# yangcaoai/CoDA_NeurIPS2023

Measured on NVIDIA H100. Metric: training scenes/sec (20k-pt SUN-RGBD synth, 256 queries), higher is better.
Workload: dtype fp32

## Files before the change

### coda_neurips2023_b200/csrc/gemm_tn32_sm90.cu

```cuda
#include "../../include/coda_gemm.h"
#include "a32_prologue.cuh"
#include "sm90_primitives.cuh"

using namespace coda;

namespace {

constexpr int BM = 128;
constexpr int BKR = 32;
constexpr int NS = 2;
constexpr int RAW_STAGES = 2, PL_STAGES = 3;
constexpr int TW = 8;
constexpr int TN32_THREADS = 288;

struct TN32Maps {
  CUtensorMap a, a2, b;
};

struct TN32Params {
  long long rows;
  int m, n;
  int a_mode, b_mode;
  const float *a_scale, *a_shift, *a_alpha, *a_beta;
  const float *dpooled;
  const unsigned char *argmax;
  int group;
  const float *b_scale, *b_shift;
  float *a_colsum;
  float *partial;
  float *c;
  long long ldc;
  int ksplit;
};

template <int BN>
__global__ void __launch_bounds__(TN32_THREADS, 1)
gemm_tn32_kernel(const __grid_constant__ TN32Maps maps, const TN32Params P) {
  constexpr int RAW_A = BKR * BM * 4;
  constexpr int RAW_B = BKR * BN * 4;
  constexpr int RAW_X = 1024;
  constexpr int RAW_STAGE = 2 * RAW_A + RAW_B + RAW_X;
  constexpr int PL_A = BKR * BM * 2;
  constexpr int PL_B = BKR * BN * 2;
  constexpr int PL_STAGE = NS * (PL_A + PL_B);
  extern __shared__ __align__(1024) unsigned char smem_raw[];
  unsigned char *smem = smem_align1024(smem_raw);
  unsigned char *raw_ring = smem;
  unsigned char *pl_ring = smem + (size_t)RAW_STAGES * RAW_STAGE;
  __shared__ __align__(8) uint64_t raw_full[RAW_STAGES], raw_empty[RAW_STAGES];
  __shared__ __align__(16) float s_colsum[TW][BM];

  const int warp = threadIdx.x >> 5, lane = threadIdx.x & 31;
  const int tiles_n = (P.n + BN - 1) / BN;
  const int tile = blockIdx.x / P.ksplit, ks = blockIdx.x % P.ksplit;
  const int m0 = (tile / tiles_n) * BM, n0 = (tile % tiles_n) * BN;
  const long long nkb_total = (P.rows + BKR - 1) / BKR;
  const long long per = (nkb_total + P.ksplit - 1) / P.ksplit;
  const long long kb0 = (long long)ks * per;
  const long long nkb = max(0ll, min(per, nkb_total - kb0));
  const bool two_in = P.a_mode == CODA_A32_BN_BWD;

  if (threadIdx.x == 0) {
    for (int s = 0; s < RAW_STAGES; ++s) { mbar_init(&raw_full[s], 1); mbar_init(&raw_empty[s], TW); }
    mbar_fence_init_cluster();
  }
  __syncthreads();

  if (warp == 8) {
    if (lane == 0) {
      prefetch_tmap(&maps.a);
      prefetch_tmap(&maps.b);
      if (two_in) prefetch_tmap(&maps.a2);
    }
    const bool pooled = P.a_mode == CODA_A32_BN_BWD_POOLED || P.a_mode == CODA_A32_BN_BWD_POOLED_PRE;
    const uint32_t bytes = (uint32_t)(RAW_A * (two_in ? 2 : 1) + RAW_B + (pooled ? 640 : 0));
    const long long ngroups = pooled ? P.rows / P.group : 0;
    for (long long i = 0; i < nkb; ++i) {
      const int rs = (int)(i % RAW_STAGES);
      mbar_wait(&raw_empty[rs], (uint32_t)((i / RAW_STAGES) & 1) ^ 1u);
      if (elect_one_sync()) {
        unsigned char *st = raw_ring + (size_t)rs * RAW_STAGE;
        const int r0 = (int)((kb0 + i) * BKR);
        mbar_arrive_expect_tx(&raw_full[rs], bytes);
        if (pooled) {
          long long g = (long long)r0 / P.group;
          if (g >= ngroups) g = ngroups - 1;
          bulk_load_1d(st + 2 * RAW_A + RAW_B, P.dpooled + g * P.m + m0, 512, &raw_full[rs]);
          bulk_load_1d(st + 2 * RAW_A + RAW_B + 512, P.argmax + g * P.m + m0, 128, &raw_full[rs]);
        }
#pragma unroll
        for (int g = 0; g < BM / 32; ++g) tma_load_3d(st + g * 4096, &maps.a, &raw_full[rs], m0 + g * 32, r0, 0);
        if (two_in) {
#pragma unroll
          for (int g = 0; g < BM / 32; ++g) tma_load_3d(st + RAW_A + g * 4096, &maps.a2, &raw_full[rs], m0 + g * 32, r0, 0);
        }
#pragma unroll
        for (int g = 0; g < BN / 32; ++g) tma_load_3d(st + 2 * RAW_A + g * 4096, &maps.b, &raw_full[rs], n0 + g * 32, r0, 0);
      }
      __syncwarp();
    }
    return;
  }

  const int tw = warp;
  const int wg = warp >> 2;
  const bool want_colsum = P.a_colsum != nullptr && n0 == 0;
  float4 csum = make_float4(0.f, 0.f, 0.f, 0.f);
  const int ca = m0 + lane * 4;
  float4 sa = make_float4(0.f, 0.f, 0.f, 0.f), ta = sa, al = sa, be = sa;
  if (P.a_mode != CODA_A32_PLAIN && ca < P.m) {
    sa = __ldg(reinterpret_cast<const float4 *>(P.a_scale + ca));
    ta = __ldg(reinterpret_cast<const float4 *>(P.a_shift + ca));
    al = __ldg(reinterpret_cast<const float4 *>(P.a_alpha + ca));
    be = __ldg(reinterpret_cast<const float4 *>(P.a_beta + ca));
  }
  constexpr int B_CHUNKS = BN / 4, B_RPP = 32 / B_CHUNKS;
  const int bch = lane % B_CHUNKS, brow_off = lane / B_CHUNKS;
  const int cb = n0 + bch * 4;
  float4 sb = make_float4(0.f, 0.f, 0.f, 0.f), tb = sb;
  if (P.b_mode == CODA_A32_AFFINE_RELU && cb < P.n) {
    sb = __ldg(reinterpret_cast<const float4 *>(P.b_scale + cb));
    tb = __ldg(reinterpret_cast<const float4 *>(P.b_shift + cb));
  }
  const bool a_col_ok = ca < P.m;
  const bool pooled_mode = P.a_mode == CODA_A32_BN_BWD_POOLED || P.a_mode == CODA_A32_BN_BWD_POOLED_PRE;
  int rem0 = pooled_mode ? (int)((kb0 * BKR) % P.group) : 0;
  int rs = 0, ps = 0;
  uint32_t raw_par = 0;
  float acc[BN / 2];
  for (long long i = 0; i < nkb; ++i) {
    mbar_wait_relaxed(&raw_full[rs], raw_par);
    const unsigned char *raw = raw_ring + (size_t)rs * RAW_STAGE;
    unsigned char *pl = pl_ring + (size_t)ps * PL_STAGE;
    const long long r0 = (kb0 + i) * BKR;
    const bool tail = r0 + BKR > P.rows;
#pragma unroll
      for (int j = 0; j < BKR / TW; ++j) {
        const int r = tw + j * TW;
        const long long grow = r0 + r;
        const uint32_t roff = (uint32_t)(lane >> 3) * 4096u + (uint32_t)r * 128u + (uint32_t)(((lane & 7) ^ (r & 7)) << 4);
        float4 y = *reinterpret_cast<const float4 *>(raw + roff);
        float4 o = y;
        if (P.a_mode == CODA_A32_BN_BWD) {
          const float4 d = *reinterpret_cast<const float4 *>(raw + RAW_A + roff);
          o.x = a32::bn_bwd(y.x, d.x, sa.x, ta.x, al.x, be.x);
          o.y = a32::bn_bwd(y.y, d.y, sa.y, ta.y, al.y, be.y);
          o.z = a32::bn_bwd(y.z, d.z, sa.z, ta.z, al.z, be.z);
          o.w = a32::bn_bwd(y.w, d.w, sa.w, ta.w, al.w, be.w);
        } else if (P.a_mode == CODA_A32_BN_BWD_POOLED_PRE) {
          const int gi = rem0 + r;
          const float4 d = *reinterpret_cast<const float4 *>(raw + 2 * RAW_A + RAW_B + lane * 16);
          const uchar4 id = *reinterpret_cast<const uchar4 *>(raw + 2 * RAW_A + RAW_B + 512 + lane * 4);
          o.x = a32::bn_bwd_pooled_pre(y.x, d.x, id.x == gi, al.x, be.x);
          o.y = a32::bn_bwd_pooled_pre(y.y, d.y, id.y == gi, al.y, be.y);
          o.z = a32::bn_bwd_pooled_pre(y.z, d.z, id.z == gi, al.z, be.z);
          o.w = a32::bn_bwd_pooled_pre(y.w, d.w, id.w == gi, al.w, be.w);
        } else if (P.a_mode == CODA_A32_BN_BWD_POOLED) {
          const int gi = rem0 + r;
          const float4 d = *reinterpret_cast<const float4 *>(raw + 2 * RAW_A + RAW_B + lane * 16);
          const uchar4 id = *reinterpret_cast<const uchar4 *>(raw + 2 * RAW_A + RAW_B + 512 + lane * 4);
          o.x = a32::bn_bwd_pooled(y.x, d.x, id.x == gi, sa.x, ta.x, al.x, be.x);
          o.y = a32::bn_bwd_pooled(y.y, d.y, id.y == gi, sa.y, ta.y, al.y, be.y);
          o.z = a32::bn_bwd_pooled(y.z, d.z, id.z == gi, sa.z, ta.z, al.z, be.z);
          o.w = a32::bn_bwd_pooled(y.w, d.w, id.w == gi, sa.w, ta.w, al.w, be.w);
        }
        if (tail && grow >= P.rows) o = make_float4(0.f, 0.f, 0.f, 0.f);
        if (want_colsum) { csum.x += o.x; csum.y += o.y; csum.z += o.z; csum.w += o.w; }
        const int col = lane * 4;
        split_store4<NS>(o, reinterpret_cast<__nv_bfloat16 *>(pl + (col >> 6) * (BKR * 128) + r * 128 +
                                                              ((((col & 63) >> 3) ^ (r & 7)) << 4) + ((col & 7) >> 2) * 8),
                         PL_A / 2);
      }
#pragma unroll
      for (int j = 0; j < BKR / (TW * B_RPP); ++j) {
        const int r = (tw + j * TW) * B_RPP + brow_off;
        const long long grow = r0 + r;
        const uint32_t roff = (uint32_t)(bch >> 3) * 4096u + (uint32_t)r * 128u + (uint32_t)(((bch & 7) ^ (r & 7)) << 4);
        float4 v = *reinterpret_cast<const float4 *>(raw + 2 * RAW_A + roff);
        if (P.b_mode == CODA_A32_AFFINE_RELU) {
          v.x = a32::affine_relu(v.x, sb.x, tb.x); v.y = a32::affine_relu(v.y, sb.y, tb.y);
          v.z = a32::affine_relu(v.z, sb.z, tb.z); v.w = a32::affine_relu(v.w, sb.w, tb.w);
        }
        if (tail && grow >= P.rows) v = make_float4(0.f, 0.f, 0.f, 0.f);
        const int col = bch * 4;
        split_store4<NS>(v, reinterpret_cast<__nv_bfloat16 *>(pl + NS * PL_A + (col >> 6) * (BKR * 128) + r * 128 +
                                                              ((((col & 63) >> 3) ^ (r & 7)) << 4) + ((col & 7) >> 2) * 8),
                         PL_B / 2);
      }
      fence_proxy_async_smem();
      __syncwarp();
      if (lane == 0) mbar_arrive(&raw_empty[rs]);
      bar_sync(1, 256);
      acc_fence(acc);
      wgmma_fence();
#pragma unroll
      for (int p = 0; p < n_products(NS); ++p) {
        const uint64_t ad = gmma_desc_mn_sw128(pl + prod_a(NS, p) * PL_A + wg * (BKR * 128), BKR * 128);
        const uint64_t bd = gmma_desc_mn_sw128(pl + NS * PL_A + prod_b(NS, p) * PL_B, BKR * 128);
#pragma unroll
        for (int kk = 0; kk < BKR / 16; ++kk)
          Wgmma<BN, false>::template ss<1, 1>(acc, gmma_desc_advance(ad, kk * 16 * 128), gmma_desc_advance(bd, kk * 16 * 128),
                                              (i | p | kk) != 0);
      }
      wgmma_commit();
      wgmma_wait<1>();
      acc_fence(acc);
      if (++rs == RAW_STAGES) { rs = 0; raw_par ^= 1u; }
      if (++ps == PL_STAGES) ps = 0;
      if (pooled_mode) { rem0 += BKR; if (rem0 >= P.group) rem0 -= P.group; }
  }
  wgmma_wait<0>();
  acc_fence(acc);
  if (nkb == 0) acc_zero(acc);
  *reinterpret_cast<float4 *>(&s_colsum[tw][lane * 4]) = csum;
  {
    const int g = lane >> 2, t4 = lane & 3;
    float *slot = P.partial + ((long long)tile * P.ksplit + ks) * (BM * BN);
#pragma unroll
    for (int i = 0; i < 2; ++i) {
      const int rl = wg * 64 + (warp & 3) * 16 + g + 8 * i, row = m0 + rl;
      float *crow = P.c + (size_t)row * P.ldc;
#pragma unroll
      for (int c = 0; c < BN / 8; ++c) {
        const int col = n0 + c * 8 + 2 * t4;
        const float2 v = make_float2(acc[c * 4 + i * 2], acc[c * 4 + i * 2 + 1]);
        if (P.ksplit > 1) *reinterpret_cast<float2 *>(slot + (size_t)rl * BN + c * 8 + 2 * t4) = v;
        else if (row < P.m && col < P.n) *reinterpret_cast<float2 *>(crow + col) = v;
      }
    }
  }
  bar_sync(1, 256);
  if (P.a_colsum && n0 == 0 && threadIdx.x < BM) {
    float cs = 0.f;
#pragma unroll
    for (int w = 0; w < TW; ++w) cs += s_colsum[w][threadIdx.x];
    if (P.ksplit > 1) {
      const int tiles_m = (P.m + BM - 1) / BM;
      P.partial[(long long)tiles_m * (tiles_n * P.ksplit) * (BM * BN) + ((long long)(m0 / BM) * P.ksplit + ks) * BM +
                threadIdx.x] = cs;
    } else if (m0 + (int)threadIdx.x < P.m) {
      P.a_colsum[m0 + threadIdx.x] = cs;
    }
  }
}

__global__ void __launch_bounds__(256)
colsum_reduce_kernel(const float *__restrict__ parts, int ksplit, int m, float *__restrict__ a_colsum) {
  const int col = blockIdx.x * blockDim.x + threadIdx.x;
  if (col >= m) return;
  const float *src = parts + ((long long)(col / BM) * ksplit) * BM + col % BM;
  float v = 0.f;
  for (int k = 0; k < ksplit; ++k) v += src[(long long)k * BM];
  a_colsum[col] = v;
}

template <int BN>
int launch_tn32(const TN32Maps &maps, TN32Params P, float *c, long long ldc, cudaStream_t s) {
  constexpr size_t smem = (size_t)RAW_STAGES * (2 * BKR * BM * 4 + BKR * BN * 4 + 1024) +
                          (size_t)PL_STAGES * NS * (BKR * BM * 2 + BKR * BN * 2) + 1024;
  static_assert(smem <= 227 * 1024, "smem budget");
  constexpr auto kern = gemm_tn32_kernel<BN>;
  if (const int st = raise_smem_limit<kern>((int)smem)) return st;
  const int num_sms = sm_count();
  const int tiles = ((P.m + BM - 1) / BM) * ((P.n + BN - 1) / BN);
  const long long nkb_total = (P.rows + BKR - 1) / BKR;
  int ksplit = num_sms / tiles;
  if (ksplit < 1) ksplit = 1;
  if (ksplit > nkb_total / 4) ksplit = (int)(nkb_total / 4 > 0 ? nkb_total / 4 : 1);
  P.ksplit = ksplit;
  const int tiles_m = (P.m + BM - 1) / BM;
  if (ksplit > 1) {
    const int st = split_scratch((size_t)tiles * ksplit * BM * BN + (size_t)tiles_m * ksplit * BM, s, &P.partial);
    if (st != CODA_OK) return st;
  }
  kern<<<tiles * ksplit, TN32_THREADS, smem, s>>>(maps, P);
  if (ksplit > 1) {
    const long long total = (long long)P.m * P.n;
    const long long blocks = (total + 255) / 256;
    splitk_reduce_kernel<<<(unsigned)(blocks < 8 * num_sms ? blocks : 8 * num_sms), 256, 0, s>>>(
        P.partial, ksplit, P.m, P.n, 1, BM, BN, nullptr, c, ldc, 0);
    if (P.a_colsum)
      colsum_reduce_kernel<<<(P.m + 255) / 256, 256, 0, s>>>(P.partial + (size_t)tiles * ksplit * BM * BN, ksplit, P.m,
                                                            P.a_colsum);
  }
  return launch_status();
}

}

extern "C" {

int coda_gemm_tn32(long long rows, int m, int n, const float *a, long long lda, int a_mode, const float *a_scale,
                   const float *a_shift, const float *a_alpha, const float *a_beta, const float *a2, long long lda2,
                   const unsigned char *a_argmax, int a_group, const float *b, long long ldb, int b_mode,
                   const float *b_scale, const float *b_shift, float *c, long long ldc, float *a_colsum, void *stream) {
  if (rows <= 0 || m <= 0 || n <= 0 || !a || !b || !c) return CODA_EINVAL;
  if ((lda & 3) || (ldb & 3) || (ldc & 3) || (m & 3) || (n & 3)) return CODA_EINVAL;
  if (((uintptr_t)a | (uintptr_t)b | (uintptr_t)c) & 15) return CODA_EINVAL;
  if (a_mode != CODA_A32_PLAIN && a_mode != CODA_A32_BN_BWD && a_mode != CODA_A32_BN_BWD_POOLED &&
      a_mode != CODA_A32_BN_BWD_POOLED_PRE)
    return CODA_EINVAL;
  if (b_mode != CODA_A32_PLAIN && b_mode != CODA_A32_AFFINE_RELU) return CODA_EINVAL;
  if (a_mode != CODA_A32_PLAIN && (!a_scale || !a_shift || !a_alpha || !a_beta || !a2 || ((uintptr_t)a2 & 15))) return CODA_EINVAL;
  if (a_mode == CODA_A32_BN_BWD && (lda2 & 3)) return CODA_EINVAL;
  if ((a_mode == CODA_A32_BN_BWD_POOLED || a_mode == CODA_A32_BN_BWD_POOLED_PRE) &&
      (!a_argmax || a_group < 32 || a_group > 256 || a_group % 32 != 0 || rows % a_group != 0 || m % 128 != 0))
    return CODA_EINVAL;
  if (b_mode == CODA_A32_AFFINE_RELU && (!b_scale || !b_shift)) return CODA_EINVAL;
  TN32Maps maps;
  int st = make_tmap_f32_box(&maps.a, a, m, rows, lda, 32, BKR);
  if (st != CODA_OK) return st;
  maps.a2 = maps.a;
  if (a_mode == CODA_A32_BN_BWD) {
    st = make_tmap_f32_box(&maps.a2, a2, m, rows, lda2, 32, BKR);
    if (st != CODA_OK) return st;
  }
  st = make_tmap_f32_box(&maps.b, b, n, rows, ldb, 32, BKR);
  if (st != CODA_OK) return st;
  TN32Params P;
  P.rows = rows; P.m = m; P.n = n; P.a_mode = a_mode; P.b_mode = b_mode;
  P.a_scale = a_scale; P.a_shift = a_shift; P.a_alpha = a_alpha; P.a_beta = a_beta;
  P.dpooled = a2; P.argmax = a_argmax; P.group = a_group; P.b_scale = b_scale; P.b_shift = b_shift; P.a_colsum = a_colsum; P.partial = nullptr; P.c = c; P.ldc = ldc; P.ksplit = 1;
  cudaStream_t s = (cudaStream_t)stream;
  if (n <= 64) return launch_tn32<64>(maps, P, c, ldc, s);
  return launch_tn32<128>(maps, P, c, ldc, s);
}

}
```

### coda_neurips2023_b200/csrc/sm90_primitives.cuh

```cuda
#pragma once
#include <cuda.h>
#include <cuda_bf16.h>
#include <cuda_fp16.h>

#include <mutex>

#include "coda_common.cuh"
#include "operand_split.cuh"
#include "wgmma_ops.cuh"

namespace coda {

typedef CUresult (*EncodeTiledFn)(CUtensorMap *, CUtensorMapDataType, cuuint32_t, void *, const cuuint64_t *,
                                  const cuuint64_t *, const cuuint32_t *, const cuuint32_t *, CUtensorMapInterleave,
                                  CUtensorMapSwizzle, CUtensorMapL2promotion, CUtensorMapFloatOOBfill);

inline EncodeTiledFn encode_tiled_fn() {
  static thread_local bool ctx_bound = false;
  if (!ctx_bound) {
    cudaFree(nullptr);
    ctx_bound = true;
  }
  static EncodeTiledFn fn = nullptr;
  if (!fn) {
    void *p = nullptr;
    cudaDriverEntryPointQueryResult q;
    if (cudaGetDriverEntryPoint("cuTensorMapEncodeTiled", &p, cudaEnableDefault, &q) == cudaSuccess &&
        q == cudaDriverEntryPointSuccess)
      fn = (EncodeTiledFn)p;
  }
  return fn;
}

inline int make_tmap_k_major_16b(CUtensorMap *map, const void *base, int is_fp16, long long k, long long rows,
                                 long long batch, long long row_stride, long long batch_stride, int box_rows) {
  EncodeTiledFn fn = encode_tiled_fn();
  if (!fn) return CODA_EINVAL;
  cuuint64_t gdim[3] = {(cuuint64_t)k, (cuuint64_t)rows, (cuuint64_t)batch};
  cuuint64_t gstride[2] = {(cuuint64_t)row_stride * 2, (cuuint64_t)(batch > 1 ? batch_stride : row_stride * rows) * 2};
  cuuint32_t box[3] = {64, (cuuint32_t)box_rows, 1};
  cuuint32_t estr[3] = {1, 1, 1};
  CUresult r = fn(map, is_fp16 ? CU_TENSOR_MAP_DATA_TYPE_FLOAT16 : CU_TENSOR_MAP_DATA_TYPE_BFLOAT16, 3,
                  const_cast<void *>(base), gdim, gstride, box, estr, CU_TENSOR_MAP_INTERLEAVE_NONE,
                  CU_TENSOR_MAP_SWIZZLE_128B, CU_TENSOR_MAP_L2_PROMOTION_L2_256B, CU_TENSOR_MAP_FLOAT_OOB_FILL_NONE);
  return r == CUDA_SUCCESS ? CODA_OK : CODA_EINVAL;
}

inline int make_tmap_f32_box(CUtensorMap *map, const void *base, long long cols, long long rows, long long row_stride,
                             int box_cols, int box_rows) {
  EncodeTiledFn fn = encode_tiled_fn();
  if (!fn) return CODA_EINVAL;
  cuuint64_t gdim[3] = {(cuuint64_t)cols, (cuuint64_t)rows, 1};
  cuuint64_t gstride[2] = {(cuuint64_t)row_stride * 4, (cuuint64_t)row_stride * rows * 4};
  cuuint32_t box[3] = {(cuuint32_t)box_cols, (cuuint32_t)box_rows, 1};
  cuuint32_t estr[3] = {1, 1, 1};
  CUresult r = fn(map, CU_TENSOR_MAP_DATA_TYPE_FLOAT32, 3, const_cast<void *>(base), gdim, gstride, box, estr,
                  CU_TENSOR_MAP_INTERLEAVE_NONE, CU_TENSOR_MAP_SWIZZLE_128B, CU_TENSOR_MAP_L2_PROMOTION_L2_256B,
                  CU_TENSOR_MAP_FLOAT_OOB_FILL_NONE);
  return r == CUDA_SUCCESS ? CODA_OK : CODA_EINVAL;
}

inline int sm_count() {
  static int n = 0;
  if (!n) {
    int dev = 0;
    cudaGetDevice(&dev);
    cudaDeviceGetAttribute(&n, cudaDevAttrMultiProcessorCount, dev);
    if (n <= 0) n = 132;
  }
  return n;
}

inline int split_scratch(size_t floats, cudaStream_t s, float **out) {
  static std::mutex mu;
  static float *buf[64] = {};
  static size_t cap[64] = {};
  int dev = 0;
  cudaGetDevice(&dev);
  if (dev < 0 || dev >= 64) return CODA_EINVAL;
  std::lock_guard<std::mutex> lock(mu);
  if (cap[dev] < floats) {
    cudaStreamCaptureStatus cs = cudaStreamCaptureStatusNone;
    if (cudaStreamIsCapturing(s, &cs) != cudaSuccess || cs != cudaStreamCaptureStatusNone) return CODA_ETOOLARGE;
    const size_t want = floats > 2 * cap[dev] ? floats : 2 * cap[dev];
    float *p = nullptr;
    cudaError_t e = cudaMalloc(&p, want * sizeof(float));
    if (e != cudaSuccess) return (int)e;
    buf[dev] = p;
    cap[dev] = want;
  }
  *out = buf[dev];
  return CODA_OK;
}

static __global__ void __launch_bounds__(256)
splitk_reduce_kernel(const float *__restrict__ partial, int ksplit, int m, int n, int batch, int bm, int bn,
                     const float *__restrict__ bias, float *__restrict__ c, long long ldc, long long c_batch_stride) {
  const long long total = (long long)batch * m * n;
  const int tiles_m = (m + bm - 1) / bm, tiles_n = (n + bn - 1) / bn;
  for (long long i = (long long)blockIdx.x * blockDim.x + threadIdx.x; i < total; i += (long long)gridDim.x * blockDim.x) {
    const int col = (int)(i % n);
    const long long t = i / n;
    const int row = (int)(t % m), b = (int)(t / m);
    const long long tile = ((long long)b * tiles_m + row / bm) * tiles_n + col / bn;
    const float *src = partial + (tile * ksplit) * bm * bn + (long long)(row % bm) * bn + col % bn;
    float v = bias ? __ldg(bias + col) : 0.f;
    for (int k = 0; k < ksplit; ++k) v += src[(long long)k * bm * bn];
    c[(size_t)b * c_batch_stride + (size_t)row * ldc + col] = v;
  }
}

__device__ __forceinline__ void prefetch_tmap(const CUtensorMap *m) {
  asm volatile("prefetch.tensormap [%0];" ::"l"(reinterpret_cast<uint64_t>(m)) : "memory");
}

__device__ __forceinline__ void tma_load_3d(void *smem_dst, const CUtensorMap *map, uint64_t *bar, int c0, int c1,
                                            int c2) {
  asm volatile(
      "cp.async.bulk.tensor.3d.shared::cluster.global.mbarrier::complete_tx::bytes [%0], [%1, {%3, %4, %5}], [%2];"
      ::"r"(smem_u32(smem_dst)), "l"(reinterpret_cast<uint64_t>(map)), "r"(smem_u32(bar)), "r"(c0), "r"(c1), "r"(c2)
      : "memory");
}

__device__ __forceinline__ void bulk_load_1d(void *smem_dst, const void *gsrc, uint32_t bytes, uint64_t *bar) {
  asm volatile("cp.async.bulk.shared::cluster.global.mbarrier::complete_tx::bytes [%0], [%1], %2, [%3];"
               ::"r"(smem_u32(smem_dst)), "l"(reinterpret_cast<uint64_t>(gsrc)), "r"(bytes), "r"(smem_u32(bar))
               : "memory");
}

__device__ __forceinline__ void fence_proxy_async_smem() { asm volatile("fence.proxy.async.shared::cta;" ::: "memory"); }

__device__ __forceinline__ bool elect_one_sync() {
  uint32_t pred;
  asm volatile(
      "{\n\t.reg .pred p;\n\t"
      "elect.sync _|p, 0xffffffff;\n\t"
      "selp.u32 %0, 1, 0, p;\n\t}"
      : "=r"(pred));
  return pred != 0;
}

__device__ __forceinline__ void wgmma_fence() { asm volatile("wgmma.fence.sync.aligned;" ::: "memory"); }
__device__ __forceinline__ void wgmma_commit() { asm volatile("wgmma.commit_group.sync.aligned;" ::: "memory"); }
template <int N>
__device__ __forceinline__ void wgmma_wait() { asm volatile("wgmma.wait_group.sync.aligned %0;" ::"n"(N) : "memory"); }
template <int R>
__device__ __forceinline__ void acc_fence(float (&d)[R]) {
#pragma unroll
  for (int i = 0; i < R; ++i) asm volatile("" : "+f"(d[i])::"memory");
}
template <int R>
__device__ __forceinline__ void acc_zero(float (&d)[R]) {
#pragma unroll
  for (int i = 0; i < R; ++i) d[i] = 0.f;
}
template <int N>
__device__ __forceinline__ void setmaxnreg_dec() { asm volatile("setmaxnreg.dec.sync.aligned.u32 %0;" ::"n"(N)); }
template <int N>
__device__ __forceinline__ void setmaxnreg_inc() { asm volatile("setmaxnreg.inc.sync.aligned.u32 %0;" ::"n"(N)); }
__device__ __forceinline__ void bar_sync(int id, int threads) {
  asm volatile("bar.sync %0, %1;" ::"r"(id), "r"(threads) : "memory");
}
__device__ __forceinline__ void bar_arrive(int id, int threads) {
  asm volatile("bar.arrive %0, %1;" ::"r"(id), "r"(threads) : "memory");
}

__device__ __forceinline__ uint64_t gmma_desc_k_sw128(const void *tile) {
  uint64_t d = 0;
  d |= (uint64_t)((smem_u32(tile) & 0x3FFFF) >> 4);
  d |= (uint64_t)1 << 16;
  d |= (uint64_t)(1024 >> 4) << 32;
  d |= (uint64_t)1 << 62;
  return d;
}
__device__ __forceinline__ uint64_t gmma_desc_mn_sw128(const void *tile, uint32_t lbo = 8192) {
  uint64_t d = 0;
  d |= (uint64_t)((smem_u32(tile) & 0x3FFFF) >> 4);
  d |= (uint64_t)(lbo >> 4) << 16;
  d |= (uint64_t)(1024 >> 4) << 32;
  d |= (uint64_t)1 << 62;
  return d;
}

__device__ __forceinline__ uint64_t gmma_desc_advance(uint64_t desc, uint32_t bytes) { return desc + (bytes >> 4); }

__device__ __forceinline__ unsigned char *smem_align1024(unsigned char *smem_raw) {
  return reinterpret_cast<unsigned char *>((reinterpret_cast<uintptr_t>(smem_raw) + 1023) & ~(uintptr_t)1023);
}

}
```

Baseline: 199.0.

## Fuse split-K reduction into last CTA and deepen raw ring for single-input modes

Adds per-tile atomic counters so the last split-K CTA for each tile sums the partial slices and writes C (and the column sums) directly, removing the separate splitk_reduce kernel launch when ksplit is small. The kernel is also templated on whether a second A input is present. Single-input modes therefore no longer reserve a second A slot in every raw stage and can use up to four raw stages within the shared-memory budget. The cost is serialized reduction work in one CTA per tile, extra atomics and fences, and counters that must be reset to zero after each use.

Measured after the change: 199.9, median of 6. No clear change (+0.5%).

```diff
diff --git a/coda_neurips2023_b200/csrc/gemm_tn32_sm90.cu b/coda_neurips2023_b200/csrc/gemm_tn32_sm90.cu
--- a/coda_neurips2023_b200/csrc/gemm_tn32_sm90.cu
+++ b/coda_neurips2023_b200/csrc/gemm_tn32_sm90.cu
@@ -9,9 +9,27 @@
 constexpr int BM = 128;
 constexpr int BKR = 32;
 constexpr int NS = 2;
-constexpr int RAW_STAGES = 2, PL_STAGES = 3;
+constexpr int PL_STAGES = 3;
 constexpr int TW = 8;
 constexpr int TN32_THREADS = 288;
+constexpr int FUSED_REDUCE_MAX_SPLITS = 11;
+
+template <int BN, bool TWO_IN>
+struct TN32Smem {
+  static constexpr int RAW_A = BKR * BM * 4;
+  static constexpr int RAW_B = BKR * BN * 4;
+  static constexpr int RAW_X = 1024;
+  static constexpr int A_SLOTS = TWO_IN ? 2 : 1;
+  static constexpr int RAW_STAGE = A_SLOTS * RAW_A + RAW_B + RAW_X;
+  static constexpr int PL_A = BKR * BM * 2;
+  static constexpr int PL_B = BKR * BN * 2;
+  static constexpr int PL_STAGE = NS * (PL_A + PL_B);
+  static constexpr int STATIC = TW * BM * 4 + 1024;
+  static constexpr int FREE = 227 * 1024 - STATIC - 1024 - PL_STAGES * PL_STAGE;
+  static constexpr int RAW_STAGES = TWO_IN ? 2 : FREE / RAW_STAGE > 4 ? 4 : FREE / RAW_STAGE;
+  static constexpr size_t BYTES = (size_t)RAW_STAGES * RAW_STAGE + (size_t)PL_STAGES * PL_STAGE + 1024;
+  static_assert(RAW_STAGES >= 2, "smem budget");
+};
 
 struct TN32Maps {
   CUtensorMap a, a2, b;
@@ -28,27 +46,27 @@
   const float *b_scale, *b_shift;
   float *a_colsum;
   float *partial;
+  unsigned *counters;
   float *c;
   long long ldc;
   int ksplit;
 };
 
-template <int BN>
+template <int BN, bool TWO_IN>
 __global__ void __launch_bounds__(TN32_THREADS, 1)
 gemm_tn32_kernel(const __grid_constant__ TN32Maps maps, const TN32Params P) {
-  constexpr int RAW_A = BKR * BM * 4;
-  constexpr int RAW_B = BKR * BN * 4;
-  constexpr int RAW_X = 1024;
-  constexpr int RAW_STAGE = 2 * RAW_A + RAW_B + RAW_X;
-  constexpr int PL_A = BKR * BM * 2;
-  constexpr int PL_B = BKR * BN * 2;
-  constexpr int PL_STAGE = NS * (PL_A + PL_B);
+  using L = TN32Smem<BN, TWO_IN>;
+  constexpr int RAW_A = L::RAW_A, RAW_B = L::RAW_B, RAW_STAGE = L::RAW_STAGE, RAW_STAGES = L::RAW_STAGES;
+  constexpr int RAW_BOFF = L::A_SLOTS * RAW_A;
+  constexpr int RAW_XOFF = RAW_BOFF + RAW_B;
+  constexpr int PL_A = L::PL_A, PL_B = L::PL_B, PL_STAGE = L::PL_STAGE;
   extern __shared__ __align__(1024) unsigned char smem_raw[];
   unsigned char *smem = smem_align1024(smem_raw);
   unsigned char *raw_ring = smem;
   unsigned char *pl_ring = smem + (size_t)RAW_STAGES * RAW_STAGE;
   __shared__ __align__(8) uint64_t raw_full[RAW_STAGES], raw_empty[RAW_STAGES];
   __shared__ __align__(16) float s_colsum[TW][BM];
+  __shared__ int s_last;
 
   const int warp = threadIdx.x >> 5, lane = threadIdx.x & 31;
   const int tiles_n = (P.n + BN - 1) / BN;
@@ -58,7 +76,7 @@
   const long long per = (nkb_total + P.ksplit - 1) / P.ksplit;
   const long long kb0 = (long long)ks * per;
   const long long nkb = max(0ll, min(per, nkb_total - kb0));
-  const bool two_in = P.a_mode == CODA_A32_BN_BWD;
+  constexpr bool two_in = TWO_IN;
 
   if (threadIdx.x == 0) {
     for (int s = 0; s < RAW_STAGES; ++s) { mbar_init(&raw_full[s], 1); mbar_init(&raw_empty[s], TW); }
@@ -85,8 +103,8 @@
         if (pooled) {
           long long g = (long long)r0 / P.group;
           if (g >= ngroups) g = ngroups - 1;
-          bulk_load_1d(st + 2 * RAW_A + RAW_B, P.dpooled + g * P.m + m0, 512, &raw_full[rs]);
-          bulk_load_1d(st + 2 * RAW_A + RAW_B + 512, P.argmax + g * P.m + m0, 128, &raw_full[rs]);
+          bulk_load_1d(st + RAW_XOFF, P.dpooled + g * P.m + m0, 512, &raw_full[rs]);
+          bulk_load_1d(st + RAW_XOFF + 512, P.argmax + g * P.m + m0, 128, &raw_full[rs]);
         }
 #pragma unroll
         for (int g = 0; g < BM / 32; ++g) tma_load_3d(st + g * 4096, &maps.a, &raw_full[rs], m0 + g * 32, r0, 0);
@@ -95,7 +113,7 @@
           for (int g = 0; g < BM / 32; ++g) tma_load_3d(st + RAW_A + g * 4096, &maps.a2, &raw_full[rs], m0 + g * 32, r0, 0);
         }
 #pragma unroll
-        for (int g = 0; g < BN / 32; ++g) tma_load_3d(st + 2 * RAW_A + g * 4096, &maps.b, &raw_full[rs], n0 + g * 32, r0, 0);
+        for (int g = 0; g < BN / 32; ++g) tma_load_3d(st + RAW_BOFF + g * 4096, &maps.b, &raw_full[rs], n0 + g * 32, r0, 0);
       }
       __syncwarp();
     }
@@ -141,7 +159,7 @@
         const uint32_t roff = (uint32_t)(lane >> 3) * 4096u + (uint32_t)r * 128u + (uint32_t)(((lane & 7) ^ (r & 7)) << 4);
         float4 y = *reinterpret_cast<const float4 *>(raw + roff);
         float4 o = y;
-        if (P.a_mode == CODA_A32_BN_BWD) {
+        if (two_in) {
           const float4 d = *reinterpret_cast<const float4 *>(raw + RAW_A + roff);
           o.x = a32::bn_bwd(y.x, d.x, sa.x, ta.x, al.x, be.x);
           o.y = a32::bn_bwd(y.y, d.y, sa.y, ta.y, al.y, be.y);
@@ -149,16 +167,16 @@
           o.w = a32::bn_bwd(y.w, d.w, sa.w, ta.w, al.w, be.w);
         } else if (P.a_mode == CODA_A32_BN_BWD_POOLED_PRE) {
           const int gi = rem0 + r;
-          const float4 d = *reinterpret_cast<const float4 *>(raw + 2 * RAW_A + RAW_B + lane * 16);
-          const uchar4 id = *reinterpret_cast<const uchar4 *>(raw + 2 * RAW_A + RAW_B + 512 + lane * 4);
+          const float4 d = *reinterpret_cast<const float4 *>(raw + RAW_XOFF + lane * 16);
+          const uchar4 id = *reinterpret_cast<const uchar4 *>(raw + RAW_XOFF + 512 + lane * 4);
           o.x = a32::bn_bwd_pooled_pre(y.x, d.x, id.x == gi, al.x, be.x);
           o.y = a32::bn_bwd_pooled_pre(y.y, d.y, id.y == gi, al.y, be.y);
           o.z = a32::bn_bwd_pooled_pre(y.z, d.z, id.z == gi, al.z, be.z);
           o.w = a32::bn_bwd_pooled_pre(y.w, d.w, id.w == gi, al.w, be.w);
         } else if (P.a_mode == CODA_A32_BN_BWD_POOLED) {
           const int gi = rem0 + r;
-          const float4 d = *reinterpret_cast<const float4 *>(raw + 2 * RAW_A + RAW_B + lane * 16);
-          const uchar4 id = *reinterpret_cast<const uchar4 *>(raw + 2 * RAW_A + RAW_B + 512 + lane * 4);
+          const float4 d = *reinterpret_cast<const float4 *>(raw + RAW_XOFF + lane * 16);
+          const uchar4 id = *reinterpret_cast<const uchar4 *>(raw + RAW_XOFF + 512 + lane * 4);
           o.x = a32::bn_bwd_pooled(y.x, d.x, id.x == gi, sa.x, ta.x, al.x, be.x);
           o.y = a32::bn_bwd_pooled(y.y, d.y, id.y == gi, sa.y, ta.y, al.y, be.y);
           o.z = a32::bn_bwd_pooled(y.z, d.z, id.z == gi, sa.z, ta.z, al.z, be.z);
@@ -176,7 +194,7 @@
         const int r = (tw + j * TW) * B_RPP + brow_off;
         const long long grow = r0 + r;
         const uint32_t roff = (uint32_t)(bch >> 3) * 4096u + (uint32_t)r * 128u + (uint32_t)(((bch & 7) ^ (r & 7)) << 4);
-        float4 v = *reinterpret_cast<const float4 *>(raw + 2 * RAW_A + roff);
+        float4 v = *reinterpret_cast<const float4 *>(raw + RAW_BOFF + roff);
         if (P.b_mode == CODA_A32_AFFINE_RELU) {
           v.x = a32::affine_relu(v.x, sb.x, tb.x); v.y = a32::affine_relu(v.y, sb.y, tb.y);
           v.z = a32::affine_relu(v.z, sb.z, tb.z); v.w = a32::affine_relu(v.w, sb.w, tb.w);
@@ -242,6 +260,43 @@
       P.a_colsum[m0 + threadIdx.x] = cs;
     }
   }
+  if (P.counters) {
+    __threadfence();
+    bar_sync(1, 256);
+    if (threadIdx.x == 0) s_last = atomicAdd(&P.counters[tile], 1u) == (unsigned)(P.ksplit - 1);
+    bar_sync(1, 256);
+    if (!s_last) return;
+    __threadfence();
+    constexpr int PER = BM * BN / 4 / 256;
+    const float *tslots = P.partial + (long long)tile * P.ksplit * (BM * BN);
+    float4 v[PER];
+#pragma unroll
+    for (int j = 0; j < PER; ++j) v[j] = make_float4(0.f, 0.f, 0.f, 0.f);
+    for (int k = 0; k < P.ksplit; ++k) {
+      const float4 *src = reinterpret_cast<const float4 *>(tslots + (long long)k * (BM * BN)) + threadIdx.x;
+#pragma unroll
+      for (int j = 0; j < PER; ++j) {
+        const float4 p = __ldcg(src + j * 256);
+        v[j].x += p.x; v[j].y += p.y; v[j].z += p.z; v[j].w += p.w;
+      }
+    }
+#pragma unroll
+    for (int j = 0; j < PER; ++j) {
+      const int e = (threadIdx.x + j * 256) * 4;
+      const int row = m0 + e / BN, col = n0 + e % BN;
+      if (row < P.m && col < P.n)
+        *reinterpret_cast<float4 *>(P.c + (size_t)row * P.ldc + col) = v[j];
+    }
+    if (P.a_colsum && n0 == 0 && threadIdx.x < BM && m0 + (int)threadIdx.x < P.m) {
+      const int tiles_m = (P.m + BM - 1) / BM;
+      const float *cslots = P.partial + (long long)tiles_m * (tiles_n * P.ksplit) * (BM * BN) +
+                            (long long)(m0 / BM) * P.ksplit * BM + threadIdx.x;
+      float v = 0.f;
+      for (int k = 0; k < P.ksplit; ++k) v += __ldcg(cslots + (long long)k * BM);
+      P.a_colsum[m0 + threadIdx.x] = v;
+    }
+    if (threadIdx.x == 0) P.counters[tile] = 0u;
+  }
 }
 
 __global__ void __launch_bounds__(256)
@@ -254,12 +309,10 @@
   a_colsum[col] = v;
 }
 
-template <int BN>
+template <int BN, bool TWO_IN>
 int launch_tn32(const TN32Maps &maps, TN32Params P, float *c, long long ldc, cudaStream_t s) {
-  constexpr size_t smem = (size_t)RAW_STAGES * (2 * BKR * BM * 4 + BKR * BN * 4 + 1024) +
-                          (size_t)PL_STAGES * NS * (BKR * BM * 2 + BKR * BN * 2) + 1024;
-  static_assert(smem <= 227 * 1024, "smem budget");
-  constexpr auto kern = gemm_tn32_kernel<BN>;
+  constexpr size_t smem = TN32Smem<BN, TWO_IN>::BYTES;
+  constexpr auto kern = gemm_tn32_kernel<BN, TWO_IN>;
   if (const int st = raise_smem_limit<kern>((int)smem)) return st;
   const int num_sms = sm_count();
   const int tiles = ((P.m + BM - 1) / BM) * ((P.n + BN - 1) / BN);
@@ -269,12 +322,14 @@
   if (ksplit > nkb_total / 4) ksplit = (int)(nkb_total / 4 > 0 ? nkb_total / 4 : 1);
   P.ksplit = ksplit;
   const int tiles_m = (P.m + BM - 1) / BM;
+  const bool fused = ksplit > 1 && ksplit <= FUSED_REDUCE_MAX_SPLITS && tiles <= SPLIT_COUNTERS;
   if (ksplit > 1) {
-    const int st = split_scratch((size_t)tiles * ksplit * BM * BN + (size_t)tiles_m * ksplit * BM, s, &P.partial);
+    const int st = split_scratch((size_t)tiles * ksplit * BM * BN + (size_t)tiles_m * ksplit * BM, s, &P.partial,
+                                 fused ? &P.counters : nullptr);
     if (st != CODA_OK) return st;
   }
   kern<<<tiles * ksplit, TN32_THREADS, smem, s>>>(maps, P);
-  if (ksplit > 1) {
+  if (ksplit > 1 && !fused) {
     const long long total = (long long)P.m * P.n;
     const long long blocks = (total + 255) / 256;
     splitk_reduce_kernel<<<(unsigned)(blocks < 8 * num_sms ? blocks : 8 * num_sms), 256, 0, s>>>(
@@ -320,10 +375,11 @@
   TN32Params P;
   P.rows = rows; P.m = m; P.n = n; P.a_mode = a_mode; P.b_mode = b_mode;
   P.a_scale = a_scale; P.a_shift = a_shift; P.a_alpha = a_alpha; P.a_beta = a_beta;
-  P.dpooled = a2; P.argmax = a_argmax; P.group = a_group; P.b_scale = b_scale; P.b_shift = b_shift; P.a_colsum = a_colsum; P.partial = nullptr; P.c = c; P.ldc = ldc; P.ksplit = 1;
+  P.dpooled = a2; P.argmax = a_argmax; P.group = a_group; P.b_scale = b_scale; P.b_shift = b_shift; P.a_colsum = a_colsum; P.partial = nullptr; P.counters = nullptr; P.c = c; P.ldc = ldc; P.ksplit = 1;
   cudaStream_t s = (cudaStream_t)stream;
-  if (n <= 64) return launch_tn32<64>(maps, P, c, ldc, s);
-  return launch_tn32<128>(maps, P, c, ldc, s);
-}
-
-}
+  const bool two_in = a_mode == CODA_A32_BN_BWD;
+  if (n <= 64) return two_in ? launch_tn32<64, true>(maps, P, c, ldc, s) : launch_tn32<64, false>(maps, P, c, ldc, s);
+  return two_in ? launch_tn32<128, true>(maps, P, c, ldc, s) : launch_tn32<128, false>(maps, P, c, ldc, s);
+}
+
+}
diff --git a/coda_neurips2023_b200/csrc/sm90_primitives.cuh b/coda_neurips2023_b200/csrc/sm90_primitives.cuh
--- a/coda_neurips2023_b200/csrc/sm90_primitives.cuh
+++ b/coda_neurips2023_b200/csrc/sm90_primitives.cuh
@@ -71,7 +71,8 @@
   return n;
 }
 
-inline int split_scratch(size_t floats, cudaStream_t s, float **out) {
+constexpr int SPLIT_COUNTERS = 1024;
+inline int split_scratch(size_t floats, cudaStream_t s, float **out, unsigned **counters = nullptr) {
   static std::mutex mu;
   static float *buf[64] = {};
   static size_t cap[64] = {};
@@ -84,12 +85,15 @@
     if (cudaStreamIsCapturing(s, &cs) != cudaSuccess || cs != cudaStreamCaptureStatusNone) return CODA_ETOOLARGE;
     const size_t want = floats > 2 * cap[dev] ? floats : 2 * cap[dev];
     float *p = nullptr;
-    cudaError_t e = cudaMalloc(&p, want * sizeof(float));
+    cudaError_t e = cudaMalloc(&p, (want + SPLIT_COUNTERS) * sizeof(float));
+    if (e != cudaSuccess) return (int)e;
+    e = cudaMemsetAsync(p, 0, SPLIT_COUNTERS * sizeof(unsigned), s);
     if (e != cudaSuccess) return (int)e;
     buf[dev] = p;
     cap[dev] = want;
   }
-  *out = buf[dev];
+  *out = buf[dev] + SPLIT_COUNTERS;
+  if (counters) *counters = reinterpret_cast<unsigned *>(buf[dev]);
   return CODA_OK;
 }
 
```

## Split TN32 GEMM into transform and MMA warpgroups with register reallocation

Applied to the files above, without the earlier changes.

Moves the wgmma work out of the eight transform warps into a dedicated MMA warpgroup. The groups hand off through new pl_full/pl_empty mbarriers, so fp32-to-bf16 conversion of the next tile can overlap tensor-core work on the current one instead of sitting behind a named barrier. setmaxnreg redistributes registers among producer, transform and MMA warps, and the raw/plain stage counts are rebalanced from 2/3 to 3/2. The cost is more threads, only two converted stages of slack, and a larger static shared-memory footprint.

New measurement: 199.1 before, 199.1 after, median of 6. About the same (-0.0%).

```diff
diff --git a/coda_neurips2023_b200/csrc/gemm_tn32_sm90.cu b/coda_neurips2023_b200/csrc/gemm_tn32_sm90.cu
--- a/coda_neurips2023_b200/csrc/gemm_tn32_sm90.cu
+++ b/coda_neurips2023_b200/csrc/gemm_tn32_sm90.cu
@@ -9,9 +9,11 @@
 constexpr int BM = 128;
 constexpr int BKR = 32;
 constexpr int NS = 2;
-constexpr int RAW_STAGES = 2, PL_STAGES = 3;
+constexpr int RAW_STAGES = 3, PL_STAGES = 2;
 constexpr int TW = 8;
-constexpr int TN32_THREADS = 288;
+constexpr int MMA_WARP0 = 8, PRODUCER_WARP = 12;
+constexpr int TN32_THREADS = 512;
+constexpr int PRODUCER_REGS = 40, TRANSFORM_REGS = 112, MMA_REGS = 232;
 
 struct TN32Maps {
   CUtensorMap a, a2, b;
@@ -47,7 +49,7 @@
   unsigned char *smem = smem_align1024(smem_raw);
   unsigned char *raw_ring = smem;
   unsigned char *pl_ring = smem + (size_t)RAW_STAGES * RAW_STAGE;
-  __shared__ __align__(8) uint64_t raw_full[RAW_STAGES], raw_empty[RAW_STAGES];
+  __shared__ __align__(8) uint64_t raw_full[RAW_STAGES], raw_empty[RAW_STAGES], pl_full[PL_STAGES], pl_empty[PL_STAGES];
   __shared__ __align__(16) float s_colsum[TW][BM];
 
   const int warp = threadIdx.x >> 5, lane = threadIdx.x & 31;
@@ -62,11 +64,14 @@
 
   if (threadIdx.x == 0) {
     for (int s = 0; s < RAW_STAGES; ++s) { mbar_init(&raw_full[s], 1); mbar_init(&raw_empty[s], TW); }
+    for (int s = 0; s < PL_STAGES; ++s) { mbar_init(&pl_full[s], TW); mbar_init(&pl_empty[s], 4); }
     mbar_fence_init_cluster();
   }
   __syncthreads();
 
-  if (warp == 8) {
+  if (warp >= PRODUCER_WARP) {
+    setmaxnreg_dec<PRODUCER_REGS>();
+    if (warp != PRODUCER_WARP) return;
     if (lane == 0) {
       prefetch_tmap(&maps.a);
       prefetch_tmap(&maps.b);
@@ -102,8 +107,63 @@
     return;
   }
 
+  if (warp >= MMA_WARP0) {
+    setmaxnreg_inc<MMA_REGS>();
+    float acc[2][BN / 2];
+    int ps = 0, prev = 0;
+    uint32_t pl_par = 0;
+    for (long long i = 0; i < nkb; ++i) {
+      mbar_wait(&pl_full[ps], pl_par);
+      const unsigned char *pl = pl_ring + (size_t)ps * PL_STAGE;
+      acc_fence(acc[0]);
+      acc_fence(acc[1]);
+      wgmma_fence();
+#pragma unroll
+      for (int p = 0; p < n_products(NS); ++p) {
+        const uint64_t bd = gmma_desc_mn_sw128(pl + NS * PL_A + prod_b(NS, p) * PL_B, BKR * 128);
+#pragma unroll
+        for (int h = 0; h < 2; ++h) {
+          const uint64_t ad = gmma_desc_mn_sw128(pl + prod_a(NS, p) * PL_A + h * (BKR * 128), BKR * 128);
+#pragma unroll
+          for (int kk = 0; kk < BKR / 16; ++kk)
+            Wgmma<BN, false>::template ss<1, 1>(acc[h], gmma_desc_advance(ad, kk * 16 * 128),
+                                                gmma_desc_advance(bd, kk * 16 * 128), (i | p | kk) != 0);
+        }
+      }
+      wgmma_commit();
+      wgmma_wait<1>();
+      acc_fence(acc[0]);
+      acc_fence(acc[1]);
+      if (i > 0 && lane == 0) mbar_arrive(&pl_empty[prev]);
+      prev = ps;
+      if (++ps == PL_STAGES) { ps = 0; pl_par ^= 1u; }
+    }
+    wgmma_wait<0>();
+    acc_fence(acc[0]);
+    acc_fence(acc[1]);
+    if (nkb == 0) { acc_zero(acc[0]); acc_zero(acc[1]); }
+    const int g = lane >> 2, t4 = lane & 3;
+    float *slot = P.partial + ((long long)tile * P.ksplit + ks) * (BM * BN);
+#pragma unroll
+    for (int h = 0; h < 2; ++h) {
+#pragma unroll
+      for (int i = 0; i < 2; ++i) {
+        const int rl = h * 64 + (warp - MMA_WARP0) * 16 + g + 8 * i, row = m0 + rl;
+        float *crow = P.c + (size_t)row * P.ldc;
+#pragma unroll
+        for (int c = 0; c < BN / 8; ++c) {
+          const int col = n0 + c * 8 + 2 * t4;
+          const float2 v = make_float2(acc[h][c * 4 + i * 2], acc[h][c * 4 + i * 2 + 1]);
+          if (P.ksplit > 1) *reinterpret_cast<float2 *>(slot + (size_t)rl * BN + c * 8 + 2 * t4) = v;
+          else if (row < P.m && col < P.n) *reinterpret_cast<float2 *>(crow + col) = v;
+        }
+      }
+    }
+    return;
+  }
+
+  setmaxnreg_dec<TRANSFORM_REGS>();
   const int tw = warp;
-  const int wg = warp >> 2;
   const bool want_colsum = P.a_colsum != nullptr && n0 == 0;
   float4 csum = make_float4(0.f, 0.f, 0.f, 0.f);
   const int ca = m0 + lane * 4;
@@ -126,9 +186,9 @@
   const bool pooled_mode = P.a_mode == CODA_A32_BN_BWD_POOLED || P.a_mode == CODA_A32_BN_BWD_POOLED_PRE;
   int rem0 = pooled_mode ? (int)((kb0 * BKR) % P.group) : 0;
   int rs = 0, ps = 0;
-  uint32_t raw_par = 0;
-  float acc[BN / 2];
+  uint32_t raw_par = 0, pl_par = 0;
   for (long long i = 0; i < nkb; ++i) {
+    mbar_wait_relaxed(&pl_empty[ps], pl_par ^ 1u);
     mbar_wait_relaxed(&raw_full[rs], raw_par);
     const unsigned char *raw = raw_ring + (size_t)rs * RAW_STAGE;
     unsigned char *pl = pl_ring + (size_t)ps * PL_STAGE;
@@ -189,47 +249,16 @@
       }
       fence_proxy_async_smem();
       __syncwarp();
-      if (lane == 0) mbar_arrive(&raw_empty[rs]);
-      bar_sync(1, 256);
-      acc_fence(acc);
-      wgmma_fence();
-#pragma unroll
-      for (int p = 0; p < n_products(NS); ++p) {
-        const uint64_t ad = gmma_desc_mn_sw128(pl + prod_a(NS, p) * PL_A + wg * (BKR * 128), BKR * 128);
-        const uint64_t bd = gmma_desc_mn_sw128(pl + NS * PL_A + prod_b(NS, p) * PL_B, BKR * 128);
-#pragma unroll
-        for (int kk = 0; kk < BKR / 16; ++kk)
-          Wgmma<BN, false>::template ss<1, 1>(acc, gmma_desc_advance(ad, kk * 16 * 128), gmma_desc_advance(bd, kk * 16 * 128),
-                                              (i | p | kk) != 0);
-      }
-      wgmma_commit();
-      wgmma_wait<1>();
-      acc_fence(acc);
+      if (lane == 0) {
+        mbar_arrive(&raw_empty[rs]);
+        mbar_arrive(&pl_full[ps]);
+      }
       if (++rs == RAW_STAGES) { rs = 0; raw_par ^= 1u; }
-      if (++ps == PL_STAGES) ps = 0;
+      if (++ps == PL_STAGES) { ps = 0; pl_par ^= 1u; }
       if (pooled_mode) { rem0 += BKR; if (rem0 >= P.group) rem0 -= P.group; }
   }
-  wgmma_wait<0>();
-  acc_fence(acc);
-  if (nkb == 0) acc_zero(acc);
   *reinterpret_cast<float4 *>(&s_colsum[tw][lane * 4]) = csum;
-  {
-    const int g = lane >> 2, t4 = lane & 3;
-    float *slot = P.partial + ((long long)tile * P.ksplit + ks) * (BM * BN);
-#pragma unroll
-    for (int i = 0; i < 2; ++i) {
-      const int rl = wg * 64 + (warp & 3) * 16 + g + 8 * i, row = m0 + rl;
-      float *crow = P.c + (size_t)row * P.ldc;
-#pragma unroll
-      for (int c = 0; c < BN / 8; ++c) {
-        const int col = n0 + c * 8 + 2 * t4;
-        const float2 v = make_float2(acc[c * 4 + i * 2], acc[c * 4 + i * 2 + 1]);
-        if (P.ksplit > 1) *reinterpret_cast<float2 *>(slot + (size_t)rl * BN + c * 8 + 2 * t4) = v;
-        else if (row < P.m && col < P.n) *reinterpret_cast<float2 *>(crow + col) = v;
-      }
-    }
-  }
-  bar_sync(1, 256);
+  bar_sync(1, TW * 32);
   if (P.a_colsum && n0 == 0 && threadIdx.x < BM) {
     float cs = 0.f;
 #pragma unroll
@@ -258,7 +287,7 @@
 int launch_tn32(const TN32Maps &maps, TN32Params P, float *c, long long ldc, cudaStream_t s) {
   constexpr size_t smem = (size_t)RAW_STAGES * (2 * BKR * BM * 4 + BKR * BN * 4 + 1024) +
                           (size_t)PL_STAGES * NS * (BKR * BM * 2 + BKR * BN * 2) + 1024;
-  static_assert(smem <= 227 * 1024, "smem budget");
+  static_assert(smem + sizeof(float) * TW * BM <= 227 * 1024, "smem budget (dynamic + the static column sums)");
   constexpr auto kern = gemm_tn32_kernel<BN>;
   if (const int st = raise_smem_limit<kern>((int)smem)) return st;
   const int num_sms = sm_count();
```
